# MiloszKrajewski/K4os.Compression.LZ4

Measured on AMD Instinct MI355X. Metric: GiB/s encode+decode on batched 64 KiB blocks; bit-exact vs C# ref, higher is better.
Workload: dtype u8

## Files before the change

### include/k4lz4.h

```cpp
#ifndef K4LZ4_H
#define K4LZ4_H

#include <stddef.h>
#include <stdint.h>

#ifdef __cplusplus
extern "C" {
#endif

#define K4LZ4_API __attribute__((visibility("default")))
#define K4LZ4_VERSION 100

typedef struct k4lz4_ctx k4lz4_ctx;

enum k4lz4_status {
    K4LZ4_OK = 0,
    K4LZ4_E_HIP = -1,
    K4LZ4_E_ARG = -2,
    K4LZ4_E_NOMEM = -3,
    K4LZ4_E_NO_DEVICE = -4,
    K4LZ4_E_UNSUPPORTED = -5
};

enum k4lz4_level {
// ... 21 lines not shown

K4LZ4_API int k4lz4_ctx_create(k4lz4_ctx **out, int device);
K4LZ4_API void k4lz4_ctx_destroy(k4lz4_ctx *ctx);
K4LZ4_API const char *k4lz4_last_error(const k4lz4_ctx *ctx);
K4LZ4_API int k4lz4_ctx_device(const k4lz4_ctx *ctx);
K4LZ4_API int k4lz4_synchronize(k4lz4_ctx *ctx, void *stream);
K4LZ4_API int k4lz4_ctx_reserve_hc(k4lz4_ctx *ctx, int64_t totalSrcBytes, int32_t longestBlock);
K4LZ4_API int k4lz4_host_register(void *ptr, size_t bytes);
K4LZ4_API int k4lz4_host_unregister(void *ptr);
K4LZ4_API int k4lz4_selftest_chains(k4lz4_ctx *ctx, int waves, int rounds, uint32_t seed, uint32_t mismatches[3]);
enum k4lz4_decode_kernel {
    K4LZ4_DECODE_KERNEL_NONE = 0,
    K4LZ4_DECODE_KERNEL_PAIR2 = 1,
    K4LZ4_DECODE_KERNEL_PAIR = 2,
    K4LZ4_DECODE_KERNEL_SINGLE = 3,
    K4LZ4_DECODE_KERNEL_DENSE = 4,
    K4LZ4_DECODE_KERNEL_PROF = 5,
    K4LZ4_DECODE_KERNEL_UNPICKLE_PAIR2 = 9,
    K4LZ4_DECODE_KERNEL_UNPICKLE_PAIR = 10,
    K4LZ4_DECODE_KERNEL_UNPICKLE_SINGLE = 11,
    K4LZ4_DECODE_KERNEL_PACE = 64
};
K4LZ4_API int k4lz4_last_decode_kernel(const k4lz4_ctx *ctx);

K4LZ4_API void k4lz4_set_enforce32(int on);
K4LZ4_API int k4lz4_get_enforce32(void);
K4LZ4_API int k4lz4_compress_bound(int n);

K4LZ4_API int k4lz4_last_status(void);
K4LZ4_API int k4lz4_compress_fast(const uint8_t *src, uint8_t *dst, int srcLen, int dstCap, int acceleration);
K4LZ4_API int k4lz4_compress_hc(const uint8_t *src, uint8_t *dst, int srcLen, int dstCap, int level);
K4LZ4_API int k4lz4_decompress_safe(const uint8_t *src, uint8_t *dst, int srcLen, int dstCap);
K4LZ4_API int k4lz4_decompress_safe_partial(const uint8_t *src, uint8_t *dst, int srcLen, int targetLen);
K4LZ4_API int k4lz4_decompress_safe_using_dict(const uint8_t *src, uint8_t *dst, int srcLen, int dstCap,
                                               const uint8_t *dict, int dictLen);

K4LZ4_API int k4lz4_encode_batch(k4lz4_ctx *ctx, const uint8_t *src, const uint64_t *srcOff, const int32_t *srcLen,
                                 uint8_t *dst, const uint64_t *dstOff, const int32_t *dstCap, int32_t *outLen,
                                 int64_t n, int level, int flags);
K4LZ4_API int k4lz4_decode_batch(k4lz4_ctx *ctx, const uint8_t *src, const uint64_t *srcOff, const int32_t *srcLen,
                                 uint8_t *dst, const uint64_t *dstOff, const int32_t *dstCap, int32_t *outLen,
                                 int64_t n, int flags);

K4LZ4_API int k4lz4_encode_batch_device(k4lz4_ctx *ctx, const uint8_t *src, const uint64_t *srcOff,
                                        const int32_t *srcLen, uint8_t *dst, const uint64_t *dstOff,
                                        const int32_t *dstCap, int32_t *outLen, int64_t n, int level, int flags,
// ... 470 lines not shown
```

### k4os/compression/lz4_amd/_native.py

```python
from __future__ import annotations

import ctypes as C
import os
import threading

PKG_DIR = os.path.dirname(os.path.abspath(__file__))
LIB_PATH = os.path.join(PKG_DIR, "libk4lz4.so")

K4LZ4_OK = 0
E_HIP, E_ARG, E_NOMEM, E_NO_DEVICE, E_UNSUPPORTED = -1, -2, -3, -4, -5
FLAG_RAW_RETURN = 1
FLAG_PICKLE_WRITER = 2
FLAG_NO_REORDER = 4
FLAG_REORDER = 8
FLAG_NO_SPLIT = 16
FLAG_PARTIAL = 32
FLAG_X32 = 128
FLAG_ALLOW_COPY = 64
FLAG_SEGMENTS = 256
DECODE_KERNEL_NONE, DECODE_KERNEL_PAIR2, DECODE_KERNEL_PAIR, DECODE_KERNEL_SINGLE, DECODE_KERNEL_DENSE, DECODE_KERNEL_PROF = 0, 1, 2, 3, 4, 5
DECODE_KERNEL_UNPICKLE_PAIR2, DECODE_KERNEL_UNPICKLE_PAIR, DECODE_KERNEL_UNPICKLE_SINGLE = 9, 10, 11
DECODE_KERNEL_PACE = 64

_u8p = C.c_void_p
_BATCH = [C.c_void_p, _u8p, C.c_void_p, C.c_void_p, _u8p, C.c_void_p, C.c_void_p, C.c_void_p, C.c_int64]
_FWRITE = [C.c_void_p, C.c_void_p, _u8p, C.c_void_p, _u8p, C.c_void_p, C.c_void_p, _u8p, C.c_void_p, C.c_void_p, C.c_void_p]
_FREAD = [C.c_void_p] * 11
_LEGACY_ENC = [C.c_void_p, _u8p, C.c_void_p, C.c_void_p, C.c_int64, C.c_int, C.c_int, C.c_int, _u8p, C.c_void_p, C.c_void_p, C.c_void_p]

SYMBOLS = {
    "k4lz4_version": (C.c_int, []),
    "k4lz4_device_count": (C.c_int, []),
    "k4lz4_recommended_min_batch": (C.c_int64, [C.c_int, C.c_int32, C.c_double]),
    "k4lz4_ctx_create": (C.c_int, [C.POINTER(C.c_void_p), C.c_int]),
    "k4lz4_ctx_destroy": (None, [C.c_void_p]),
    "k4lz4_last_error": (C.c_char_p, [C.c_void_p]),
    "k4lz4_ctx_device": (C.c_int, [C.c_void_p]),
    "k4lz4_synchronize": (C.c_int, [C.c_void_p, C.c_void_p]),
    "k4lz4_ctx_reserve_hc": (C.c_int, [C.c_void_p, C.c_int64, C.c_int]),
    "k4lz4_host_register": (C.c_int, [C.c_void_p, C.c_size_t]),
    "k4lz4_host_unregister": (C.c_int, [C.c_void_p]),
    "k4lz4_selftest_chains": (C.c_int, [C.c_void_p, C.c_int, C.c_int, C.c_uint32, C.POINTER(C.c_uint32)]),
    "k4lz4_last_decode_kernel": (C.c_int, [C.c_void_p]),
    "k4lz4_set_enforce32": (None, [C.c_int]),
    "k4lz4_get_enforce32": (C.c_int, []),
    "k4lz4_compress_bound": (C.c_int, [C.c_int]),
    "k4lz4_last_status": (C.c_int, []),
    "k4lz4_compress_fast": (C.c_int, [_u8p, _u8p, C.c_int, C.c_int, C.c_int]),
    "k4lz4_compress_hc": (C.c_int, [_u8p, _u8p, C.c_int, C.c_int, C.c_int]),
    "k4lz4_decompress_safe": (C.c_int, [_u8p, _u8p, C.c_int, C.c_int]),
    "k4lz4_decompress_safe_partial": (C.c_int, [_u8p, _u8p, C.c_int, C.c_int]),
    "k4lz4_encode_batch": (C.c_int, _BATCH + [C.c_int, C.c_int]),
    "k4lz4_decompress_safe_using_dict": (C.c_int, [_u8p, _u8p, C.c_int, C.c_int, _u8p, C.c_int]),
    "k4lz4_decode_batch": (C.c_int, _BATCH + [C.c_int]),
    "k4lz4_decode_dict_batch": (C.c_int, _BATCH + [C.c_int, _u8p, C.c_void_p, C.c_void_p]),
    "k4lz4_decode_dict_batch_device": (C.c_int, _BATCH + [C.c_int, _u8p, C.c_void_p, C.c_void_p, C.c_void_p]),
    "k4lz4_encode_batch_device": (C.c_int, _BATCH + [C.c_int, C.c_int, C.c_void_p]),
    "k4lz4_decode_batch_device": (C.c_int, _BATCH + [C.c_int, C.c_void_p]),
    "k4lz4_pickle_bound": (C.c_int, [C.c_int]),
    "k4lz4_unpickle_size": (C.c_int, [_u8p, C.c_int]),
    "k4lz4_pickle_batch": (C.c_int, _BATCH + [C.c_int, C.c_int]),
    "k4lz4_unpickle_batch": (C.c_int, _BATCH + [C.c_int]),
    "k4lz4_pickle_batch_device": (C.c_int, _BATCH + [C.c_int, C.c_int, C.c_void_p]),
    "k4lz4_unpickle_batch_device": (C.c_int, _BATCH + [C.c_int, C.c_void_p]),
    "k4lz4_profile_batch_device": (C.c_int, [C.c_void_p, C.c_int] + _BATCH[1:] + [C.c_void_p, C.c_void_p]),
    "k4lz4_xxh32_batch": (C.c_int, [C.c_void_p, _u8p, C.c_void_p, C.c_void_p, C.c_void_p, C.c_int64, C.c_uint32]),
# ... 171 lines not shown

    @property
    def device(self) -> int:
        return self.lib.k4lz4_ctx_device(self.handle)

    def check(self, rc: int):
        if rc == K4LZ4_OK:
            return
        msg = (self.lib.k4lz4_last_error(self.handle) or b"").decode()
        if rc == E_ARG:
            raise ValueError(msg)
        if rc == E_UNSUPPORTED:
            raise NotImplementedError(msg)
        if rc == E_NOMEM:
            raise MemoryError(msg)
        raise NativeLibraryError(f"libk4lz4 error {rc}: {msg}")

    def synchronize(self, stream: int = 0):
        self.check(self.lib.k4lz4_synchronize(self.handle, C.c_void_p(stream)))

    def last_decode_kernel(self) -> int:
        return int(self.lib.k4lz4_last_decode_kernel(self.handle))

    def close(self):
        if getattr(self, "handle", None):
            self.lib.k4lz4_ctx_destroy(self.handle)
            self.handle = None

    def __del__(self):
        try:
            self.close()
        except Exception:
            pass


_tls = threading.local()


def default_context() -> Context:
    ctx = getattr(_tls, "ctx", None)
    if ctx is None:
        dev = -1
        if "LOCAL_RANK" in os.environ:
            lib = load_library()
            n = lib.k4lz4_device_count()
            if n > 0:
# ... 40 lines not shown
```

### k4os/compression/lz4_amd/csrc/k4lz4_capi.hip

```cpp
#include <hip/hip_runtime.h>
#include <stdint.h>
#include <stdio.h>
#include <stdlib.h>
#include <string.h>
#include <algorithm>
#include <atomic>
#include <memory>
#include <new>
#include <condition_variable>
#include <functional>
#include <map>
#include <mutex>
#include <string>
#include <thread>
#include <chrono>
#include <vector>

#include "../../../../include/k4lz4.h"
#include "k4lz4_decode.hpp"
#include "k4lz4_encode_fast.hpp"
#include "k4lz4_parse.hpp"
#include "k4lz4_pickle.hpp"
#include "k4lz4_segments.hpp"
#include "k4lz4_encode_hc.hpp"
// ... 74 lines not shown
    int cost_pct = 48;
    int dec_parts = 4, dec_parts_direct = 8;
    int last_decode_kernel = 0;
    int hop2_max_per_cu = 12;
    bool hc_cand_lds = true;
    int hc_cand_dynlds = 0;
    int hc_segs = 0;
    bool hc_chain_parts = true;
    int hc_mem_pct = 33;
    int pace_min_per_cu = 6;
    bool use_pace = true;
    bool prof_gtab = false;
    uint8_t *d_parse = nullptr; size_t d_parse_cap = 0;
    bool use_parse = true;
    bool parse_queue = false;
    bool hc_records = true;
    bool parse_seg = true;
    bool parse_big = true;
    bool parse_persist = true;
    bool parse_inline_emit = true;
    bool parse_migrate = true;
    bool parse_pcost = false;
    int parse_waves = 16;
    bool trace = false;
    std::vector<uint8_t> h_chain;
    uint8_t *d_chain = nullptr; size_t d_chain_cap = 0;
    hipEvent_t ev_chain = nullptr;
    uint8_t *d_fr = nullptr; size_t d_fr_cap = 0;
    uint8_t *d_fb = nullptr; size_t d_fb_cap = 0;
    uint8_t *d_lg = nullptr; size_t d_lg_cap = 0;
    uint8_t *d_frd = nullptr; size_t d_frd_cap = 0;
    uint8_t *d_lgr = nullptr; size_t d_lgr_cap = 0;
    uint8_t *d_lga = nullptr; size_t d_lga_cap = 0;
    std::vector<uint8_t> h_fw;
    uint8_t *d_fw = nullptr; size_t d_fw_cap = 0;
    hipEvent_t ev_fw = nullptr;
    struct DictScratch {
        std::vector<uint8_t> host;
        uint8_t *dev = nullptr; size_t cap = 0;
        hipEvent_t ev = nullptr;
        std::vector<uint32_t> table, kept;
    } dict_fast, dict_hc;
    uint8_t *d_dpick = nullptr; size_t d_dpick_cap = 0;
};

struct k4lz4_dict_set {
// ... 356 lines not shown
            uint64_t *d_encoff = (uint64_t *)ctx->d_pk_meta;
            int32_t *d_enccap = (int32_t *)(d_encoff + cnt);
            int32_t *d_enclen = d_enccap + cnt;
            k4::BatchArgs a{};
            a.src = src; a.srcOff = srcOff + first; a.srcLen = srcLen + first; a.dst = dst; a.dstOff = dstOff + first;
            a.dstCap = dstCap + first; a.outLen = outLen + first; a.n = cnt; a.level = level; a.accel = 1;
            a.flags = flags | (g_enforce32.load(std::memory_order_relaxed) ? K4LZ4_FLAG_X32 : 0);
            const int seg_ok = kind == KIND_PICKLE || may_cut ? FLAG_SEGMENTS_OK : 0;
            if (kind == KIND_PICKLE) hipLaunchKernelGGL(k4::k4_pickle_prep_kernel, dim3((unsigned)((cnt + 255) / 256)), dim3(256), 0, stream, a, d_encoff, d_enccap);
            else hipLaunchKernelGGL(k4::k4_wrap_prep_kernel, dim3((unsigned)((cnt + 255) / 256)), dim3(256), 0, stream, a, d_encoff, d_enccap);
            rc = launch_inner(ctx, KIND_ENCODE, src, srcOff + first, srcLen + first, dst, d_encoff, d_enccap, d_enclen, cnt, level,
                              (flags & (K4LZ4_FLAG_NO_REORDER | K4LZ4_FLAG_X32)) | K4LZ4_FLAG_RAW_RETURN | seg_ok, stream, nullptr, hostLen ? hostLen + first : nullptr);
            if (rc != K4LZ4_OK) return rc;
            if (kind == KIND_PICKLE) hipLaunchKernelGGL(k4::k4_pickle_finish_kernel, dim3((unsigned)((cnt + k4::PICKLE_FINISH_WAVES_PER_WG - 1) / k4::PICKLE_FINISH_WAVES_PER_WG)), dim3(64 * k4::PICKLE_FINISH_WAVES_PER_WG), 0, stream, a, d_enclen);
            else hipLaunchKernelGGL(k4::k4_wrap_finish_kernel, dim3((unsigned)((cnt + k4::WRAP_FINISH_WAVES_PER_WG - 1) / k4::WRAP_FINISH_WAVES_PER_WG)), dim3(64 * k4::WRAP_FINISH_WAVES_PER_WG), 0, stream, a, d_enclen);
            K4_HIP(ctx, hipGetLastError());
        }
        return K4LZ4_OK;
    }
    const bool reorder = n > 1 &&
                         (encode_like ? !(flags & K4LZ4_FLAG_NO_REORDER)
                                      : ((flags & K4LZ4_FLAG_REORDER) != 0 ||
                                         (kind == KIND_UNPICKLE && n > 64 && !(flags & K4LZ4_FLAG_NO_REORDER))));
    uint32_t *d_cost = nullptr, *d_order = nullptr, *d_hist = nullptr;
    if (reorder) {
        const size_t cnt_max = (size_t)std::min<int64_t>(chunk_max, n);
        const size_t hist_words = std::max<size_t>(2 * (size_t)k4::PCOST_BUCKETS, 2 * (size_t)k4::COST_BUCKETS + 16);
        const size_t need = cnt_max * 8 + hist_words * 4 + 64;
        if (need > ctx->d_sched_cap) K4_HIP(ctx, hipStreamSynchronize(stream));
        int rc = grow(ctx, &ctx->d_sched, &ctx->d_sched_cap, need, false);
        if (rc != K4LZ4_OK) return rc;
        d_hist = (uint32_t *)ctx->d_sched;
        d_cost = d_hist + hist_words;
        d_order = d_cost + cnt_max;
    }
    for (int64_t first = 0; first < n; first += chunk_max) {
        const int64_t cnt = std::min<int64_t>(chunk_max, n - first);
        k4::BatchArgs a{};
        a.src = src; a.srcOff = srcOff + first; a.srcLen = srcLen + first;
        a.dst = dst; a.dstOff = dstOff + first; a.dstCap = dstCap + first;
        a.outLen = outLen + first; a.n = cnt; a.level = level; a.accel = ctx->accel;
        a.flags = flags | (g_enforce32.load(std::memory_order_relaxed) ? K4LZ4_FLAG_X32 : 0);
        const bool hop2 = cnt <= (int64_t)ctx->hop2_max_per_cu * (int64_t)ctx->cu_count;
        a.prof = ctx->prof ? ctx->prof + k4::PROF_STRIDE * first : nullptr;
        a.status = ctx->d_status;
        if (((kind == KIND_ENCODE && !parse_path) || (K4_DEC_PACE && (kind == KIND_DECODE || kind == KIND_UNPICKLE))) && ctx->use_pace && ctx->d_pace && cnt > (int64_t)ctx->pace_min_per_cu * (int64_t)ctx->cu_count) {
            a.pace = ctx->d_pace;
            K4_HIP(ctx, hipMemsetAsync(a.pace, 0, k4::PACE_BYTES, stream));
        }
        k4::SegArgs sg{};
        bool seg = false;
        if (kind == KIND_ENCODE && (flags & (FLAG_SEGMENTS_OK | K4LZ4_FLAG_SEGMENTS)) && ctx->use_segments && !a.prof && !(flags & K4LZ4_FLAG_ALLOW_COPY)) {
            static_assert(k4::SEG_HDR_DWORDS * 4 == 256, "seg_first_of finds the header in front of the items");
            size_t max_items = (size_t)k4::SEG_MAX_ITEMS;
            if (hostLen) {
                size_t bound = 0;
// ... 19 lines not shown
            sg.seg_min = ctx->seg_min; sg.seg_target = ctx->seg_target; sg.seg_warm = ctx->seg_warm; sg.seg_div = ctx->seg_div; sg.seg_target_max = ctx->seg_target_max; sg.spin_max = ctx->seg_spin_max; sg.max_items = (uint32_t)max_items;
            hipLaunchKernelGGL(k4::k4_seg_plan_kernel, dim3(1), dim3(256), 0, stream, a, sg);
            a.seg_first = sg.first; a.seg_items = sg.items; a.seg_snaps = sg.snaps;
            seg = true;
        }
        auto segments_start = [&]() -> int {
            if (!seg) return K4LZ4_OK;
            K4_HIP(ctx, hipEventRecord(ctx->ev_fork, stream));
            K4_HIP(ctx, hipStreamWaitEvent(ctx->aux2, ctx->ev_fork, 0));
            hipLaunchKernelGGL(k4::k4_encode_seg_kernel, dim3((unsigned)((sg.max_items + k4::ENCODE_WAVES_PER_WG - 1) / k4::ENCODE_WAVES_PER_WG)), dim3(64 * k4::ENCODE_WAVES_PER_WG), 0, ctx->aux2, a, sg);
            K4_HIP(ctx, hipEventRecord(ctx->ev_join2, ctx->aux2));
            return K4LZ4_OK;
        };
        auto segments_join = [&]() -> int {
            if (!seg) return K4LZ4_OK;
            K4_HIP(ctx, hipStreamWaitEvent(stream, ctx->ev_join2, 0));
            hipLaunchKernelGGL(k4::k4_seg_join_kernel, dim3((unsigned)std::min<int64_t>(k4::SEG_MAX_BLOCKS, cnt)), dim3(64), 0, stream, a, sg);
            return K4LZ4_OK;
        };
        if (dd && dd->dict) {
            a.dict = dd->dict; a.dictOff = dd->off + first; a.dictLen = dd->len + first;
            a.dictMode = dd->mode ? dd->mode + first : nullptr;
        }
        if (reorder && parse_path && kind == KIND_ENCODE && ctx->parse_pcost) {
            a.cost = d_cost; a.hist = d_hist; a.order_out = d_order;
            K4_HIP(ctx, hipMemsetAsync(d_hist, 0, 2 * k4::PCOST_BUCKETS * 4, stream));
            hipLaunchKernelGGL(k4::k4_pcost_kernel, dim3((unsigned)((cnt + k4::PCOST_WAVES_PER_WG - 1) / k4::PCOST_WAVES_PER_WG)), dim3(64 * k4::PCOST_WAVES_PER_WG), 0, stream, a);
            hipLaunchKernelGGL(k4::k4_porder_kernel, dim3((unsigned)((cnt + 255) / 256)), dim3(256), 0, stream, a);
            a.order = d_order;
        }
        else if (reorder) {
            a.cost = d_cost; a.hist = d_hist; a.order_out = d_order;
            K4_HIP(ctx, hipMemsetAsync(d_hist, 0, (2 * k4::COST_BUCKETS + 16) * 4, stream));
            hipLaunchKernelGGL(k4::k4_cost_kernel, dim3((unsigned)cnt), dim3(64), 0, stream, a, encode_like ? 0 : 1,
                               kind == KIND_ENCODE && parse_path ? k4::COST_SAMPLE_PARSE : k4::COST_SAMPLE);
            const bool two_kernels = kind == KIND_ENCODE && !a.prof && cnt > 512 && !(flags & K4LZ4_FLAG_NO_SPLIT) &&
                                     cnt > 8 * (int64_t)ctx->cu_count && ctx->split_pct <= 0;
            k4::BatchArgs ao = a;
            ao.first = two_kernels ? (uint32_t)ctx->cost_pct : 0u;
            ao.total = (uint32_t)((int64_t)ctx->lds_floor_per_cu * (int64_t)ctx->cu_count);
            hipLaunchKernelGGL(k4::k4_order_kernel, dim3((unsigned)((cnt + 255) / 256)), dim3(256), 0, stream, ao, (uint32_t)lds_share(ctx, cnt));
            a.order = d_order;
            if (two_kernels) a.split = d_hist + 2 * k4::COST_BUCKETS;
        }
        const unsigned wg4 = (unsigned)((cnt + k4::DECODE_WAVES_PER_WG - 1) / k4::DECODE_WAVES_PER_WG);
        bool parse_here = kind == KIND_ENCODE && (parse_path || (parse_seg_path && (a.order || cnt == 1)));
        const bool big_ok = ctx->parse_big && ctx->parse_inline_emit;
        bool any_small = true, any_big = big_ok;
        if (parse_here && hostLen) {
            any_small = false; any_big = false;
            for (int64_t i = 0; i < cnt && !(any_small && (any_big || !big_ok)); i++) {
                const int32_t len = hostLen[first + i];
                if (len >= (int32_t)k4::PARSE_MIN_LEN && len < k4::LIMIT_64K) any_small = true;
                else if (len >= k4::LIMIT_64K && big_ok) any_big = true;
            }
            parse_here = any_small || any_big;
        }
        int64_t waves = 0, nwg = 0, nwg_seg = 0;
        const bool seg_two_step = seg && parse_here && parse_seg_path;
        bool queue = false, slot_recs = false;
        size_t o_meta = 0, o_gtab = 0;
        if (parse_here) {
            waves = std::max<int64_t>(1, std::min<int64_t>(ctx->parse_waves, (cnt + ctx->cu_count - 1) / ctx->cu_count));
            queue = (ctx->parse_queue || parse_persistent || parse_seg_path) && a.order && cnt > waves * (int64_t)ctx->cu_count;
            nwg = queue ? (int64_t)ctx->cu_count : (cnt + waves - 1) / waves;
            if (seg_two_step) nwg_seg = std::min<int64_t>(ctx->cu_count, (cnt + (int64_t)sg.max_items + k4::PARSE_MAX_WAVES - 1) / k4::PARSE_MAX_WAVES);
            slot_recs = ctx->parse_inline_emit;
            const size_t rec_slots = slot_recs ? std::max((size_t)nwg * (size_t)waves, (size_t)nwg_seg * k4::PARSE_MAX_WAVES) : (size_t)cnt;
            o_meta = rec_slots * k4::PARSE_REC_STRIDE * sizeof(uint2); o_gtab = (o_meta + (size_t)cnt * 8 + 64 + 255) & ~(size_t)255;
            const size_t need = o_gtab + std::max(waves > k4::PARSE_LDS_TABLES ? (size_t)nwg * k4::PARSE_MAX_WAVES * 16384 : 0, (size_t)nwg_seg * k4::PARSE_MAX_WAVES * 16384);
            if (need > ctx->d_parse_cap) K4_HIP(ctx, hipStreamSynchronize(stream));
            const int rcp = grow(ctx, &ctx->d_parse, &ctx->d_parse_cap, need, false);
            if (rcp != K4LZ4_OK) { std::lock_guard<std::mutex> g(g_err_mu); ctx->error.clear(); parse_here = false; }
        }
        if (parse_here) {
            k4::ParseArgs pa{};
            pa.recs = (uint2 *)ctx->d_parse; pa.meta = (uint32_t *)(ctx->d_parse + o_meta); pa.gtab = (uint32_t *)(ctx->d_parse + o_gtab);
            pa.nwg = (uint32_t)nwg;
            pa.inline_emit = ctx->parse_inline_emit ? 1u : 0u;
            pa.slot_recs = slot_recs ? 1u : 0u;
            pa.migrate = ctx->parse_migrate ? 1u : 0u;
            pa.big = any_big ? 1u : 0u;
            K4_HIP(ctx, hipMemsetAsync(pa.meta + 2 * cnt, 0, 32, stream));
            if (queue) pa.queue = pa.meta + 2 * cnt;
            pa.nbig = pa.meta + 2 * cnt + 3;
            hipLaunchKernelGGL(k4::k4_parse_kernel, dim3((unsigned)nwg), dim3((unsigned)(64 * waves)), 0, stream, a, pa);
            if (seg_two_step) {
                k4::ParseArgs pb = pa;
                pb.queue = pa.meta + 2 * cnt + 4;
                pb.nwg = (uint32_t)nwg_seg;
                hipLaunchKernelGGL(k4::k4_parse_seg_kernel, dim3((unsigned)nwg_seg), dim3(64 * k4::PARSE_MAX_WAVES), 0, stream, a, pb, sg);
            } else if (any_big) {
                k4::ParseArgs pb = pa;
                if (queue) pb.queue = pa.queue + 4;
                hipLaunchKernelGGL(k4::k4_parse_big_kernel, dim3((unsigned)nwg), dim3((unsigned)(64 * waves)), 0, stream, a, pb);
            }
            if (!pa.inline_emit)
                hipLaunchKernelGGL(k4::k4_emit_kernel, dim3((unsigned)((cnt + k4::EMIT_WAVES_PER_WG - 1) / k4::EMIT_WAVES_PER_WG)), dim3(64 * k4::EMIT_WAVES_PER_WG), 0, stream, a, pa);
            bool rest = true;
            if (hostLen) {
                rest = false;
                for (int64_t i = 0; i < cnt && !rest; i++) rest = hostLen[first + i] < (int32_t)k4::PARSE_MIN_LEN || (hostLen[first + i] >= k4::LIMIT_64K && !any_big);
            }
            if (rest)
                hipLaunchKernelGGL(k4::k4_encode_fast_rest_kernel, dim3((unsigned)((cnt + k4::ENCODE_WAVES_PER_WG - 1) / k4::ENCODE_WAVES_PER_WG)), dim3(64 * k4::ENCODE_WAVES_PER_WG), 0, stream, a, pa);
            if (seg_two_step)
                hipLaunchKernelGGL(k4::k4_seg_join_kernel, dim3((unsigned)std::min<int64_t>(k4::SEG_MAX_BLOCKS, cnt)), dim3(64), 0, stream, a, sg);
            if (flags & K4LZ4_FLAG_ALLOW_COPY)
                hipLaunchKernelGGL(k4::k4_allow_copy_kernel, dim3((unsigned)((cnt + 3) / 4)), dim3(256), 0, stream, a);
            K4_HIP(ctx, hipGetLastError());
            continue;
        }
        switch (kind) {
        case KIND_ENCODE:
            if (a.prof && !ctx->prof_stamp) {
                if (ctx->prof_gtab) {
                    if ((size_t)cnt * 16384 > ctx->d_gtab_cap) {
                        K4_HIP(ctx, hipStreamSynchronize(ctx->aux));
                        int rc2 = grow(ctx, &ctx->d_gtab, &ctx->d_gtab_cap, (size_t)cnt * 16384, false);
                        if (rc2 != K4LZ4_OK) return rc2;
                    }
                    a.gtab = (uint32_t *)ctx->d_gtab;
                }
                hipLaunchKernelGGL(k4::k4_encode_fast_prof_kernel, dim3((unsigned)cnt), dim3(64), 0, stream, a);
            }
            else if (reorder && cnt > 512 && !(flags & K4LZ4_FLAG_NO_SPLIT)) {
                const int64_t lds_slots = 8 * (int64_t)ctx->cu_count;
                const int64_t n_lds = lds_share(ctx, cnt);
                const int64_t n_g = cnt - (a.split ? std::min<int64_t>(cnt, (int64_t)ctx->lds_floor_per_cu * (int64_t)ctx->cu_count) : n_lds);
                const int64_t gchunk = 8192;
                if (n_g > 0 && (size_t)std::min(n_g, gchunk) * 16384 > ctx->d_gtab_cap) {
                    K4_HIP(ctx, hipStreamSynchronize(ctx->aux));
                    int rc2 = grow(ctx, &ctx->d_gtab, &ctx->d_gtab_cap, (size_t)std::min(n_g, gchunk) * 16384, false);
// ... 1703 lines not shown
    ctx->hc_cand_lds = getenv("K4LZ4_HC_CAND_MEM") == nullptr;
    if (const char *e = getenv("K4LZ4_HC_CAND_DYNLDS")) ctx->hc_cand_dynlds = std::max(0, std::min(65536, atoi(e)));
    if (const char *e = getenv("K4LZ4_HC_SEGS")) { const int v = atoi(e); ctx->hc_segs = v >= 4 ? 4 : (v >= 2 ? 2 : (v == 1 ? 1 : 0)); }
    if (const char *e = getenv("K4LZ4_HC_MEM_PCT")) ctx->hc_mem_pct = std::max(0, std::min(100, atoi(e)));
    ctx->use_segments = getenv("K4LZ4_NO_SEGMENTS") == nullptr;
    if (const char *e = getenv("K4LZ4_SEG_MIN")) ctx->seg_min = (uint32_t)std::max(65536 + 4096, atoi(e));
    if (const char *e = getenv("K4LZ4_SEG_TARGET")) ctx->seg_target = ctx->seg_target_max = (uint32_t)std::max(8192, atoi(e));
    if (const char *e = getenv("K4LZ4_SEG_TARGET_MAX")) ctx->seg_target_max = (uint32_t)std::max(8192, atoi(e));
    if (const char *e = getenv("K4LZ4_SEG_WARM")) ctx->seg_warm = (uint32_t)std::max(0, atoi(e));
    if (const char *e = getenv("K4LZ4_SEG_SPIN_MAX")) ctx->seg_spin_max = (uint32_t)std::max(0, atoi(e));
    if (const char *e = getenv("K4LZ4_SEG_DIV")) ctx->seg_div = (uint32_t)std::max(0, atoi(e));
    if (const char *e = getenv("K4LZ4_PICKLE_SPLIT_MIN")) ctx->pickle_split_min = std::max(0, atoi(e));
    if (const char *e = getenv("K4LZ4_STAGE_THREADS")) ctx->stage_threads = std::max(0, std::min(63, atoi(e) - 1));
    ctx->use_parse = getenv("K4LZ4_NO_PARSE") == nullptr;
    ctx->parse_queue = getenv("K4LZ4_PARSE_QUEUE") != nullptr;
    ctx->parse_persist = getenv("K4LZ4_NO_PERSIST") == nullptr;
    ctx->parse_big = getenv("K4LZ4_NO_PARSE_BIG") == nullptr;
    ctx->parse_seg = getenv("K4LZ4_NO_PARSE_SEG") == nullptr;
    ctx->hc_records = getenv("K4LZ4_NO_HC_RECORDS") == nullptr;
    ctx->parse_pcost = getenv("K4LZ4_PCOST") != nullptr;
    ctx->parse_migrate = getenv("K4LZ4_NO_MIGRATE") == nullptr;
    ctx->parse_inline_emit = getenv("K4LZ4_NO_INLINE_EMIT") == nullptr;
    if (const char *e = getenv("K4LZ4_PARSE_WAVES")) ctx->parse_waves = std::max(1, std::min(k4::PARSE_MAX_WAVES, atoi(e)));
    ctx->trace = getenv("K4LZ4_TRACE") != nullptr;
    if (e != hipSuccess) { delete ctx; return hip_fail(nullptr, e, "hipStreamCreate"); }
    *out = ctx;
    return K4LZ4_OK;
}

void k4lz4_ctx_destroy(k4lz4_ctx *ctx)
{
    if (!ctx) return;
    (void)hipSetDevice(ctx->device);
    if (ctx->stream) { (void)hipStreamSynchronize(ctx->stream); (void)hipStreamDestroy(ctx->stream); }
    if (ctx->aux) { (void)hipStreamSynchronize(ctx->aux); (void)hipStreamDestroy(ctx->aux); }
    if (ctx->aux2) { (void)hipStreamSynchronize(ctx->aux2); (void)hipStreamDestroy(ctx->aux2); }
    if (ctx->ev_join2) (void)hipEventDestroy(ctx->ev_join2);
    if (ctx->d_seg) (void)hipFree(ctx->d_seg);
    if (ctx->d_seg_first) (void)hipFree(ctx->d_seg_first);
    if (ctx->ev_fork) (void)hipEventDestroy(ctx->ev_fork);
    if (ctx->ev_join) (void)hipEventDestroy(ctx->ev_join);
    if (ctx->ev_busy) (void)hipEventDestroy(ctx->ev_busy);
    for (int b = 0; b < 2; b++) {
        if (ctx->ev_in[b]) (void)hipEventDestroy(ctx->ev_in[b]);
        if (ctx->ev_out[b]) (void)hipEventDestroy(ctx->ev_out[b]);
        if (ctx->h_in[b]) (void)hipHostFree(ctx->h_in[b]);
// ... 116 lines not shown
    ctx->hc_res_longest = (uint32_t)longestBlock;
    return K4LZ4_OK;
}

int k4lz4_selftest_chains(k4lz4_ctx *ctx, int waves, int rounds, uint32_t seed, uint32_t mismatches[3])
{
    if (!ctx || !mismatches || waves <= 0 || rounds <= 0) return fail(ctx, K4LZ4_E_ARG, "selftest: bad arguments");
    K4_HIP(ctx, hipSetDevice(ctx->device));
    uint32_t *d_res = nullptr;
    K4_HIP(ctx, hipMalloc((void **)&d_res, 3 * sizeof(uint32_t)));
    hipError_t e = hipMemsetAsync(d_res, 0, 3 * sizeof(uint32_t), ctx->stream);
    if (e == hipSuccess) {
        hipLaunchKernelGGL(k4::k4_chain_selftest_kernel, dim3((unsigned)waves), dim3(64), 0, ctx->stream, seed, rounds, d_res);
        e = hipGetLastError();
    }
    if (e == hipSuccess) e = hipMemcpyAsync(mismatches, d_res, 3 * sizeof(uint32_t), hipMemcpyDeviceToHost, ctx->stream);
    if (e == hipSuccess) e = hipStreamSynchronize(ctx->stream);
    (void)hipFree(d_res);
    K4_HIP(ctx, e);
    return K4LZ4_OK;
}

int k4lz4_last_decode_kernel(const k4lz4_ctx *ctx) { return ctx ? ctx->last_decode_kernel : K4LZ4_DECODE_KERNEL_NONE; }

int k4lz4_last_status(void) { return tl_status; }

int k4lz4_compress_bound(int n) { return n > 0x7E000000 ? 0 : n + n / 255 + 16; }

int k4lz4_compress_fast(const uint8_t *src, uint8_t *dst, int srcLen, int dstCap, int acceleration)
{
    return single(KIND_ENCODE, src, dst, srcLen, dstCap, K4LZ4_L00_FAST, acceleration);
}

int k4lz4_compress_hc(const uint8_t *src, uint8_t *dst, int srcLen, int dstCap, int level)
{
    if (level < K4LZ4_L03_HC) {
        tl_status = fail(nullptr, K4LZ4_E_ARG, "k4lz4_compress_hc: level must be L03_HC (3) or higher");
        return 0;
    }
    return single(KIND_ENCODE, src, dst, srcLen, dstCap, level);
}

int k4lz4_decompress_safe(const uint8_t *src, uint8_t *dst, int srcLen, int dstCap)
{
    return single(KIND_DECODE, src, dst, srcLen, dstCap, 0);
}
// ... 2281 lines not shown
```

### k4os/compression/lz4_amd/csrc/k4lz4_encode_fast.hpp

```cpp
#pragma once
#include "k4lz4_common.hpp"

namespace k4 {

#ifndef K4_SEG_WAVES_MIN
#define K4_SEG_WAVES_MIN 5
#endif
#ifndef K4_GTAB_DUTY
#define K4_GTAB_DUTY 3
#endif
#ifndef K4_PACE
#define K4_PACE 1
#endif

template <int TYPE> struct FastTable;

template <> struct FastTable<1> {
    uint16_t *t;
    __device__ __forceinline__ static uint32_t hash(const uint8_t *p) { return (ld32u(p) * 2654435761u) >> (32 - 13); }
    __device__ __forceinline__ static uint32_t hash_of(uint32_t seq, uint32_t) { return (seq * 2654435761u) >> (32 - 13); }
    __device__ __forceinline__ uint32_t get(uint32_t h) const { return t[h]; }
    __device__ __forceinline__ void put(uint32_t h, uint32_t pos) const { t[h] = (uint16_t)pos; }
    __device__ __forceinline__ uint32_t get_nt(uint32_t h) const
    {
// ... 769 lines not shown
    if (src_len < LIMIT_64K) return encode_fast_block<true, false, false, PAIRS, MORE, N2, GTAB>(src, src_len, dst, dst_cap, a, ldsw, lane, nullptr, false, nullptr, gtab, pace);
    if (x32) return encode_fast_block<false, false, true, PAIRS, MORE, N2, GTAB>(src, src_len, dst, dst_cap, a, ldsw, lane, nullptr, false, nullptr, gtab, pace, sr);
    return encode_fast_block<false, false, false, PAIRS, MORE, N2, GTAB>(src, src_len, dst, dst_cap, a, ldsw, lane, nullptr, false, nullptr, gtab, pace, sr);
}

__device__ __forceinline__ int codec_encode_result(int src_len, int ret, int flags)
{
    if (flags & FLAG_RAW_RETURN) return ret;
    if (src_len <= 0) return 0;
    return ret <= 0 ? -1 : ret;
}

constexpr int COST_SAMPLE = 512, COST_SAMPLE_PARSE = 256;
constexpr int COST_BUCKETS = 64;

__device__ __forceinline__ uint32_t cost_bucket(unsigned long long cost)
{
    if (cost < 4ull) return (uint32_t)cost;
    const uint32_t l = 63u - (uint32_t)__clzll(cost);
    const uint32_t bkt = 2u * l + (uint32_t)((cost >> (l - 1u)) & 1ull);
    return bkt < (uint32_t)COST_BUCKETS ? bkt : (uint32_t)COST_BUCKETS - 1u;
}

__global__ __launch_bounds__(64) void k4_cost_kernel(BatchArgs a, int by_length, int sample_bytes = COST_SAMPLE)
{
    __shared__ __attribute__((aligned(16))) uint32_t tab[ENCODE_LDS_DWORDS];
    const int lane = lane_id();
    const long long b = (long long)blockIdx.x;
    const int src_len = a.srcLen[b];
    unsigned long long cost = 0;
    if (src_len > 0) {
        if (by_length || src_len <= 64) {
            cost = (unsigned long long)src_len;
        } else {
            const int sample = src_len < sample_bytes ? src_len : sample_bytes;
            uint32_t nseq = 0;
            (void)encode_fast_block<true>(a.src + a.srcOff[b], sample, nullptr, 0x7fffffff, 1u, tab, lane, nullptr, true, &nseq);
            cost = ((unsigned long long)(nseq * 8u + (uint32_t)sample / 16u) * (unsigned long long)src_len) / (unsigned long long)sample;
        }
    }
    if (lane == 0) {
        const uint32_t bkt = cost_bucket(cost);
        a.cost[b] = bkt;
        atomicAdd(&a.hist[bkt], 1u);
    }
}

__device__ __forceinline__ unsigned long long bucket_cost(uint32_t bkt)
{
    if (bkt < 4u) return bkt ? (unsigned long long)bkt * 4ull : 1ull;
    const uint32_t l = bkt >> 1;
    return ((bkt & 1u) ? 7ull : 5ull) << (l - 1u);
}

__global__ __launch_bounds__(256) void k4_order_kernel(BatchArgs a, uint32_t lds_max = 0xffffffffu)
{
    if (blockIdx.x == 0 && threadIdx.x == 0 && a.first != 0u) {
        unsigned long long all = 0;
        for (uint32_t k = 0; k < (uint32_t)COST_BUCKETS; k++) all += (unsigned long long)a.hist[k] * bucket_cost(k);
        const unsigned long long want = all / 100ull * (unsigned long long)a.first;
        unsigned long long have = 0, cnt = 0;
        for (int k = COST_BUCKETS - 1; k >= 0 && have < want; k--) {
            const unsigned long long c = a.hist[k], w = bucket_cost((uint32_t)k);
            if (have + c * w <= want) { have += c * w; cnt += c; }
            else { const unsigned long long part = (want - have + w - 1ull) / w; cnt += part; have = want; }
        }
        const unsigned long long floor_n = (unsigned long long)a.total < (unsigned long long)a.n ? (unsigned long long)a.total : (unsigned long long)a.n;
        if (cnt < floor_n) cnt = floor_n;
        if (cnt > (unsigned long long)a.n) cnt = (unsigned long long)a.n;
        if (cnt > (unsigned long long)lds_max) cnt = (unsigned long long)lds_max;
        a.hist[2 * COST_BUCKETS] = (uint32_t)cnt;
    }
    const long long b = (long long)blockIdx.x * 256 + threadIdx.x;
    if (b >= a.n) return;
    const uint32_t bkt = a.cost[b];
    uint32_t before = 0;
    for (uint32_t k = bkt + 1u; k < (uint32_t)COST_BUCKETS; k++) before += a.hist[k];
    const uint32_t pos = before + atomicAdd(&a.hist[COST_BUCKETS + bkt], 1u);
    a.order_out[pos] = (uint32_t)b;
}

constexpr int ENCODE_WAVES_PER_WG = 2;
struct SegFirst { SegRun run; uint32_t cap; bool cut; };
__device__ __forceinline__ SegFirst seg_first_of(const BatchArgs &a, long long b)
{
    SegFirst f;
    f.cut = false; f.cap = 0u;
    f.run.begin = 0u; f.run.emit_from = 0u; f.run.stop_at = SEG_NONE; f.run.snap_pub = nullptr; f.run.snap_chk = nullptr; f.run.resume = nullptr;
    f.run.cut = 0u; f.run.stop = 0u; f.run.state = 3u; f.run.spin_max = 0u; f.run.fix = nullptr;
    if (!a.seg_first) return f;
    const int32_t it = (int32_t)uni((uint32_t)a.seg_first[b]);
    if (it < 0) return f;
    const uint32_t *w = (const uint32_t *)a.seg_items + SEG_ITEM_WORDS * (uint32_t)it;
    f.cut = true;
    f.run.spin_max = uni(((const uint32_t *)a.seg_items)[-(int)SEG_HDR_DWORDS + 3]);
    f.run.stop_at = uni(w[4]);
    f.cap = f.run.stop_at;
    f.run.snap_chk = a.seg_snaps + (size_t)(it + 1) * SEG_SNAP_DWORDS;
    f.run.fix = a.seg_snaps + (size_t)uni(((const uint32_t *)a.seg_items)[-(int)SEG_HDR_DWORDS + 7]) * SEG_SNAP_DWORDS + 4096ull * (unsigned long long)it;
    return f;
}
__device__ __forceinline__ void seg_first_done(const BatchArgs &a, long long b, const SegFirst &f, int ret, int lane)
// ... 111 lines not shown
```

Baseline: 61.54.

## Fuse cost sampling, histogram and ordering into one persistent prelude kernel

Replaces the hipMemset plus separate cost kernel plus order kernel plus parse-meta memset sequence on the parse encode path with a single grid-stride prelude kernel. Per-block histograms go to LDS, and the last workgroup, chosen by an atomic counter, does the bucket scan and scatters the order, zeroing the parse queue words as it does so. A dirty flag skips re-clearing the prelude counters between calls. This cuts launch count and per-block one-wave launches, at the cost of a serial final scatter done by one workgroup. It also adds a debug API to read back the last cost and order arrays.

```diff
diff --git a/include/k4lz4.h b/include/k4lz4.h
--- a/include/k4lz4.h
+++ b/include/k4lz4.h
@@ -67,6 +67,7 @@
     K4LZ4_DECODE_KERNEL_PACE = 64
 };
 K4LZ4_API int k4lz4_last_decode_kernel(const k4lz4_ctx *ctx);
+K4LZ4_API int64_t k4lz4_last_order(k4lz4_ctx *ctx, uint32_t *cost, uint32_t *order, int64_t cap);
 
 K4LZ4_API void k4lz4_set_enforce32(int on);
 K4LZ4_API int k4lz4_get_enforce32(void);
diff --git a/k4os/compression/lz4_amd/_native.py b/k4os/compression/lz4_amd/_native.py
--- a/k4os/compression/lz4_amd/_native.py
+++ b/k4os/compression/lz4_amd/_native.py
@@ -42,6 +42,7 @@
     "k4lz4_host_unregister": (C.c_int, [C.c_void_p]),
     "k4lz4_selftest_chains": (C.c_int, [C.c_void_p, C.c_int, C.c_int, C.c_uint32, C.POINTER(C.c_uint32)]),
     "k4lz4_last_decode_kernel": (C.c_int, [C.c_void_p]),
+    "k4lz4_last_order": (C.c_int64, [C.c_void_p, C.c_void_p, C.c_void_p, C.c_int64]),
     "k4lz4_set_enforce32": (None, [C.c_int]),
     "k4lz4_get_enforce32": (C.c_int, []),
     "k4lz4_compress_bound": (C.c_int, [C.c_int]),
@@ -259,6 +260,18 @@
     def last_decode_kernel(self) -> int:
         return int(self.lib.k4lz4_last_decode_kernel(self.handle))
 
+    def last_order(self):
+        import numpy as np
+        n = int(self.lib.k4lz4_last_order(self.handle, None, None, 0))
+        if n < 0:
+            self.check(n)
+        cost, order = np.zeros(n, np.uint32), np.zeros(n, np.uint32)
+        if n:
+            rc = int(self.lib.k4lz4_last_order(self.handle, cost.ctypes.data, order.ctypes.data, n))
+            if rc < 0:
+                self.check(rc)
+        return cost, order
+
     def close(self):
         if getattr(self, "handle", None):
             self.lib.k4lz4_ctx_destroy(self.handle)
diff --git a/k4os/compression/lz4_amd/csrc/k4lz4_capi.hip b/k4os/compression/lz4_amd/csrc/k4lz4_capi.hip
--- a/k4os/compression/lz4_amd/csrc/k4lz4_capi.hip
+++ b/k4os/compression/lz4_amd/csrc/k4lz4_capi.hip
@@ -120,6 +120,10 @@
     bool parse_migrate = true;
     bool parse_pcost = false;
     int parse_waves = 16;
+    bool parse_prelude = true;
+    int parse_sample = k4::COST_SAMPLE_PARSE;
+    bool prelude_dirty = true;
+    size_t last_cost_at = 0, last_order_at = 0; int64_t last_order_n = 0;
     bool trace = false;
     std::vector<uint8_t> h_chain;
     uint8_t *d_chain = nullptr; size_t d_chain_cap = 0;
@@ -522,16 +526,21 @@
                          (encode_like ? !(flags & K4LZ4_FLAG_NO_REORDER)
                                       : ((flags & K4LZ4_FLAG_REORDER) != 0 ||
                                          (kind == KIND_UNPICKLE && n > 64 && !(flags & K4LZ4_FLAG_NO_REORDER))));
-    uint32_t *d_cost = nullptr, *d_order = nullptr, *d_hist = nullptr;
+    uint32_t *d_cost = nullptr, *d_order = nullptr, *d_hist = nullptr, *d_prelude = nullptr;
     if (reorder) {
         const size_t cnt_max = (size_t)std::min<int64_t>(chunk_max, n);
         const size_t hist_words = std::max<size_t>(2 * (size_t)k4::PCOST_BUCKETS, 2 * (size_t)k4::COST_BUCKETS + 16);
-        const size_t need = cnt_max * 8 + hist_words * 4 + 64;
-        if (need > ctx->d_sched_cap) K4_HIP(ctx, hipStreamSynchronize(stream));
+        const size_t need = cnt_max * 8 + (hist_words + (size_t)k4::PRELUDE_WORDS) * 4 + 64;
+        if (need > ctx->d_sched_cap) {
+            K4_HIP(ctx, hipStreamSynchronize(stream));
+            ctx->prelude_dirty = true;
+            ctx->last_order_n = 0;
+        }
         int rc = grow(ctx, &ctx->d_sched, &ctx->d_sched_cap, need, false);
         if (rc != K4LZ4_OK) return rc;
         d_hist = (uint32_t *)ctx->d_sched;
-        d_cost = d_hist + hist_words;
+        d_prelude = d_hist + hist_words;
+        d_cost = d_prelude + k4::PRELUDE_WORDS;
         d_order = d_cost + cnt_max;
     }
     for (int64_t first = 0; first < n; first += chunk_max) {
@@ -597,18 +606,12 @@
             a.dict = dd->dict; a.dictOff = dd->off + first; a.dictLen = dd->len + first;
             a.dictMode = dd->mode ? dd->mode + first : nullptr;
         }
-        if (reorder && parse_path && kind == KIND_ENCODE && ctx->parse_pcost) {
-            a.cost = d_cost; a.hist = d_hist; a.order_out = d_order;
-            K4_HIP(ctx, hipMemsetAsync(d_hist, 0, 2 * k4::PCOST_BUCKETS * 4, stream));
-            hipLaunchKernelGGL(k4::k4_pcost_kernel, dim3((unsigned)((cnt + k4::PCOST_WAVES_PER_WG - 1) / k4::PCOST_WAVES_PER_WG)), dim3(64 * k4::PCOST_WAVES_PER_WG), 0, stream, a);
-            hipLaunchKernelGGL(k4::k4_porder_kernel, dim3((unsigned)((cnt + 255) / 256)), dim3(256), 0, stream, a);
-            a.order = d_order;
-        }
-        else if (reorder) {
+        const bool prelude = reorder && parse_path && kind == KIND_ENCODE && !ctx->parse_pcost && ctx->parse_prelude;
+        auto cost_and_order = [&]() -> int {
             a.cost = d_cost; a.hist = d_hist; a.order_out = d_order;
             K4_HIP(ctx, hipMemsetAsync(d_hist, 0, (2 * k4::COST_BUCKETS + 16) * 4, stream));
             hipLaunchKernelGGL(k4::k4_cost_kernel, dim3((unsigned)cnt), dim3(64), 0, stream, a, encode_like ? 0 : 1,
-                               kind == KIND_ENCODE && parse_path ? k4::COST_SAMPLE_PARSE : k4::COST_SAMPLE);
+                               kind == KIND_ENCODE && parse_path ? ctx->parse_sample : k4::COST_SAMPLE);
             const bool two_kernels = kind == KIND_ENCODE && !a.prof && cnt > 512 && !(flags & K4LZ4_FLAG_NO_SPLIT) &&
                                      cnt > 8 * (int64_t)ctx->cu_count && ctx->split_pct <= 0;
             k4::BatchArgs ao = a;
@@ -617,7 +620,18 @@
             hipLaunchKernelGGL(k4::k4_order_kernel, dim3((unsigned)((cnt + 255) / 256)), dim3(256), 0, stream, ao, (uint32_t)lds_share(ctx, cnt));
             a.order = d_order;
             if (two_kernels) a.split = d_hist + 2 * k4::COST_BUCKETS;
-        }
+            return K4LZ4_OK;
+        };
+        if (reorder && parse_path && kind == KIND_ENCODE && ctx->parse_pcost) {
+            a.cost = d_cost; a.hist = d_hist; a.order_out = d_order;
+            K4_HIP(ctx, hipMemsetAsync(d_hist, 0, 2 * k4::PCOST_BUCKETS * 4, stream));
+            hipLaunchKernelGGL(k4::k4_pcost_kernel, dim3((unsigned)((cnt + k4::PCOST_WAVES_PER_WG - 1) / k4::PCOST_WAVES_PER_WG)), dim3(64 * k4::PCOST_WAVES_PER_WG), 0, stream, a);
+            hipLaunchKernelGGL(k4::k4_porder_kernel, dim3((unsigned)((cnt + 255) / 256)), dim3(256), 0, stream, a);
+            a.order = d_order;
+        }
+        else if (prelude) a.order = d_order;
+        else if (reorder) { const int rco = cost_and_order(); if (rco != K4LZ4_OK) return rco; }
+        if (reorder) { ctx->last_cost_at = (size_t)((uint8_t *)d_cost - ctx->d_sched); ctx->last_order_at = (size_t)((uint8_t *)d_order - ctx->d_sched); ctx->last_order_n = cnt; }
         const unsigned wg4 = (unsigned)((cnt + k4::DECODE_WAVES_PER_WG - 1) / k4::DECODE_WAVES_PER_WG);
         bool parse_here = kind == KIND_ENCODE && (parse_path || (parse_seg_path && (a.order || cnt == 1)));
         const bool big_ok = ctx->parse_big && ctx->parse_inline_emit;
@@ -648,6 +662,7 @@
             const int rcp = grow(ctx, &ctx->d_parse, &ctx->d_parse_cap, need, false);
             if (rcp != K4LZ4_OK) { std::lock_guard<std::mutex> g(g_err_mu); ctx->error.clear(); parse_here = false; }
         }
+        if (prelude && !parse_here) { const int rco = cost_and_order(); if (rco != K4LZ4_OK) return rco; }
         if (parse_here) {
             k4::ParseArgs pa{};
             pa.recs = (uint2 *)ctx->d_parse; pa.meta = (uint32_t *)(ctx->d_parse + o_meta); pa.gtab = (uint32_t *)(ctx->d_parse + o_gtab);
@@ -656,7 +671,16 @@
             pa.slot_recs = slot_recs ? 1u : 0u;
             pa.migrate = ctx->parse_migrate ? 1u : 0u;
             pa.big = any_big ? 1u : 0u;
-            K4_HIP(ctx, hipMemsetAsync(pa.meta + 2 * cnt, 0, 32, stream));
+            if (prelude) {
+                if (ctx->prelude_dirty) K4_HIP(ctx, hipMemsetAsync(d_prelude, 0, k4::PRELUDE_WORDS * 4, stream));
+                ctx->prelude_dirty = true;
+                a.cost = d_cost; a.order_out = d_order;
+                const int64_t pwg = std::min<int64_t>((cnt + k4::PRELUDE_WAVES - 1) / k4::PRELUDE_WAVES, ctx->cu_count);
+                hipLaunchKernelGGL(k4::k4_prelude_kernel, dim3((unsigned)pwg), dim3(64 * k4::PRELUDE_WAVES), 0, stream, a, d_prelude,
+                                   pa.meta + 2 * cnt, ctx->parse_sample);
+                K4_HIP(ctx, hipGetLastError());
+            }
+            else K4_HIP(ctx, hipMemsetAsync(pa.meta + 2 * cnt, 0, 32, stream));
             if (queue) pa.queue = pa.meta + 2 * cnt;
             pa.nbig = pa.meta + 2 * cnt + 3;
             hipLaunchKernelGGL(k4::k4_parse_kernel, dim3((unsigned)nwg), dim3((unsigned)(64 * waves)), 0, stream, a, pa);
@@ -684,6 +708,7 @@
             if (flags & K4LZ4_FLAG_ALLOW_COPY)
                 hipLaunchKernelGGL(k4::k4_allow_copy_kernel, dim3((unsigned)((cnt + 3) / 4)), dim3(256), 0, stream, a);
             K4_HIP(ctx, hipGetLastError());
+            if (prelude) ctx->prelude_dirty = false;
             continue;
         }
         switch (kind) {
@@ -2433,6 +2458,8 @@
     ctx->parse_migrate = getenv("K4LZ4_NO_MIGRATE") == nullptr;
     ctx->parse_inline_emit = getenv("K4LZ4_NO_INLINE_EMIT") == nullptr;
     if (const char *e = getenv("K4LZ4_PARSE_WAVES")) ctx->parse_waves = std::max(1, std::min(k4::PARSE_MAX_WAVES, atoi(e)));
+    ctx->parse_prelude = getenv("K4LZ4_NO_PRELUDE") == nullptr;
+    if (const char *e = getenv("K4LZ4_PARSE_SAMPLE")) ctx->parse_sample = std::max(65, std::min(k4::COST_SAMPLE, atoi(e)));
     ctx->trace = getenv("K4LZ4_TRACE") != nullptr;
     if (e != hipSuccess) { delete ctx; return hip_fail(nullptr, e, "hipStreamCreate"); }
     *out = ctx;
@@ -2595,6 +2622,20 @@
 }
 
 int k4lz4_last_decode_kernel(const k4lz4_ctx *ctx) { return ctx ? ctx->last_decode_kernel : K4LZ4_DECODE_KERNEL_NONE; }
+
+int64_t k4lz4_last_order(k4lz4_ctx *ctx, uint32_t *cost, uint32_t *order, int64_t cap)
+{
+    if (!ctx || cap < 0 || (cap > 0 && (!cost || !order))) return fail(ctx, K4LZ4_E_ARG, "k4lz4_last_order: bad arguments");
+    K4_HIP(ctx, hipSetDevice(ctx->device));
+    if (ctx->busy) K4_HIP(ctx, hipEventSynchronize(ctx->ev_busy));
+    const int64_t n = ctx->d_sched ? ctx->last_order_n : 0;
+    const size_t bytes = (size_t)std::min(n, cap) * 4;
+    if (bytes) {
+        K4_HIP(ctx, hipMemcpy(cost, ctx->d_sched + ctx->last_cost_at, bytes, hipMemcpyDeviceToHost));
+        K4_HIP(ctx, hipMemcpy(order, ctx->d_sched + ctx->last_order_at, bytes, hipMemcpyDeviceToHost));
+    }
+    return n;
+}
 
 int k4lz4_last_status(void) { return tl_status; }
 
diff --git a/k4os/compression/lz4_amd/csrc/k4lz4_encode_fast.hpp b/k4os/compression/lz4_amd/csrc/k4lz4_encode_fast.hpp
--- a/k4os/compression/lz4_amd/csrc/k4lz4_encode_fast.hpp
+++ b/k4os/compression/lz4_amd/csrc/k4lz4_encode_fast.hpp
@@ -815,11 +815,8 @@
     return bkt < (uint32_t)COST_BUCKETS ? bkt : (uint32_t)COST_BUCKETS - 1u;
 }
 
-__global__ __launch_bounds__(64) void k4_cost_kernel(BatchArgs a, int by_length, int sample_bytes = COST_SAMPLE)
-{
-    __shared__ __attribute__((aligned(16))) uint32_t tab[ENCODE_LDS_DWORDS];
-    const int lane = lane_id();
-    const long long b = (long long)blockIdx.x;
+__device__ __forceinline__ uint32_t block_cost_bucket(const BatchArgs &a, long long b, int by_length, int sample_bytes, uint32_t *tab, int lane)
+{
     const int src_len = a.srcLen[b];
     unsigned long long cost = 0;
     if (src_len > 0) {
@@ -832,8 +829,16 @@
             cost = ((unsigned long long)(nseq * 8u + (uint32_t)sample / 16u) * (unsigned long long)src_len) / (unsigned long long)sample;
         }
     }
+    return cost_bucket(cost);
+}
+
+__global__ __launch_bounds__(64) void k4_cost_kernel(BatchArgs a, int by_length, int sample_bytes = COST_SAMPLE)
+{
+    __shared__ __attribute__((aligned(16))) uint32_t tab[ENCODE_LDS_DWORDS];
+    const int lane = lane_id();
+    const long long b = (long long)blockIdx.x;
+    const uint32_t bkt = block_cost_bucket(a, b, by_length, sample_bytes, tab, lane);
     if (lane == 0) {
-        const uint32_t bkt = cost_bucket(cost);
         a.cost[b] = bkt;
         atomicAdd(&a.hist[bkt], 1u);
     }
@@ -871,6 +876,94 @@
     for (uint32_t k = bkt + 1u; k < (uint32_t)COST_BUCKETS; k++) before += a.hist[k];
     const uint32_t pos = before + atomicAdd(&a.hist[COST_BUCKETS + bkt], 1u);
     a.order_out[pos] = (uint32_t)b;
+}
+
+constexpr int PRELUDE_WAVES = 9;
+constexpr int PRELUDE_WORDS = COST_BUCKETS + 16;
+static_assert(COST_BUCKETS == 64, "k4_prelude_kernel: one lane per bucket");
+
+__device__ __forceinline__ uint32_t agent_load(const uint32_t *p)
+{
+#ifndef K4_HOST_EMU
+    return __hip_atomic_load(p, __ATOMIC_RELAXED, __HIP_MEMORY_SCOPE_AGENT);
+#else
+    return __atomic_load_n(p, __ATOMIC_RELAXED);
+#endif
+}
+__device__ __forceinline__ void agent_store(uint32_t *p, uint32_t v)
+{
+#ifndef K4_HOST_EMU
+    __hip_atomic_store(p, v, __ATOMIC_RELAXED, __HIP_MEMORY_SCOPE_AGENT);
+#else
+    __atomic_store_n(p, v, __ATOMIC_RELAXED);
+#endif
+}
+__device__ __forceinline__ uint32_t agent_exchange(uint32_t *p, uint32_t v)
+{
+#ifndef K4_HOST_EMU
+    return __hip_atomic_exchange(p, v, __ATOMIC_RELAXED, __HIP_MEMORY_SCOPE_AGENT);
+#else
+    return __atomic_exchange_n(p, v, __ATOMIC_RELAXED);
+#endif
+}
+__device__ __forceinline__ void agent_fence()
+{
+#ifndef K4_HOST_EMU
+    __threadfence();
+#else
+    __atomic_thread_fence(__ATOMIC_SEQ_CST);
+#endif
+}
+
+__global__ __launch_bounds__(64 * PRELUDE_WAVES) void k4_prelude_kernel(BatchArgs a, uint32_t *words, uint32_t *zero8, int sample_bytes)
+{
+    __shared__ __attribute__((aligned(16))) uint32_t tabs[PRELUDE_WAVES][ENCODE_LDS_DWORDS];
+    __shared__ uint32_t h[COST_BUCKETS];
+    __shared__ uint32_t last;
+    const int lane = lane_id();
+    const uint32_t wave = uni(threadIdx.x >> 6);
+    if (threadIdx.x < (unsigned)COST_BUCKETS) h[threadIdx.x] = 0u;
+    __syncthreads();
+    const long long stride = (long long)gridDim.x * PRELUDE_WAVES;
+    for (long long b = (long long)blockIdx.x * PRELUDE_WAVES + (long long)wave; b < a.n; b += stride) {
+        const uint32_t bkt = block_cost_bucket(a, b, 0, sample_bytes, tabs[wave], lane);
+        if (lane == 0) {
+            agent_store(&a.cost[b], bkt);
+            atomicAdd(&h[bkt], 1u);
+        }
+    }
+    __syncthreads();
+    if (threadIdx.x < (unsigned)COST_BUCKETS && h[threadIdx.x] != 0u) atomicAdd(&words[threadIdx.x], h[threadIdx.x]);
+    agent_fence();
+    __syncthreads();
+    if (threadIdx.x == 0) last = atomicAdd(&words[COST_BUCKETS], 1u) == gridDim.x - 1u ? 1u : 0u;
+    __syncthreads();
+    if (last == 0u) return;
+    agent_fence();
+    if (wave == 0u) {
+        const uint32_t k = (uint32_t)COST_BUCKETS - 1u - (uint32_t)lane;
+        const uint32_t c = agent_exchange(&words[k], 0u);
+        const uint32_t incl = wave_inclusive_scan(c);
+        h[k] = incl - c;
+        if (lane == 0) agent_store(&words[COST_BUCKETS], 0u);
+        if (lane < 8 && zero8) zero8[lane] = 0u;
+    }
+    __syncthreads();
+    constexpr int PER = 8;
+    for (long long base = 0; base < a.n; base += (long long)PER * (long long)blockDim.x) {
+        uint32_t bkt[PER];
+#pragma unroll
+        for (int j = 0; j < PER; j++) {
+            const long long b = base + (long long)j * (long long)blockDim.x + (long long)threadIdx.x;
+            bkt[j] = b < a.n ? agent_load(&a.cost[b]) : 0xffffffffu;
+        }
+#pragma unroll
+        for (int j = 0; j < PER; j++) {
+            if (bkt[j] >= (uint32_t)COST_BUCKETS) continue;
+            const uint32_t pos = atomicAdd(&h[bkt[j]], 1u);
+            if ((long long)pos < a.n) a.order_out[pos] = (uint32_t)(base + (long long)j * (long long)blockDim.x + (long long)threadIdx.x);
+        }
+    }
 }
 
 constexpr int ENCODE_WAVES_PER_WG = 2;
```

Result: no change. 61.87, median of 6 (+0.5%).
